# MasterBin-IIAU/Unicorn

Hardware: NVIDIA B200
Metric: frames/sec (higher is better)
Workload: dtype bf16

## Files before the change

### include/unicorn_b200.h

```cpp
#ifndef UNICORN_B200_H_
#define UNICORN_B200_H_
#include <stdint.h>

#ifdef __cplusplus
extern "C" {
#endif

#if defined(__GNUC__)
#define UC_API __attribute__((visibility("default")))
#else
#define UC_API
#endif

#define UC_OK 0
#define UC_EINVAL (-1)
#define UC_EDRIVER (-2)
#define UC_ENODEV (-3)

#define UC_BF16 0
#define UC_F32 1
#define UC_F16 2

#define UC_ACT_NONE 0
#define UC_ACT_RELU 1
// ... 19 lines not shown
  void* y;
  int ldy;
  int y_dtype;
  int block_n;
  void* gn_stats;
  int gn_groups;
  const void* row_stats;
  const float* col_s;
  float row_eps;
} UcConv2d;
UC_API int uc_conv2d(const UcConv2d* d, void* stream);

UC_API int uc_stem_ln(const void* img, int img_is_u8_hwc, const float* w48, const float* bias, const float* lnw, const float* lnb,
                      void* out_bf16, int B, int H, int W, int C0, float eps, void* stream);

UC_API int uc_dwconv7_ln(const void* x_bf16, const float* w49, const float* bias, const float* lnw, const float* lnb,
                         void* y_bf16, int B, int H, int W, int C, float eps, void* stream);

UC_API int uc_dwconv7(const void* x_bf16, const float* w49, const float* bias, void* y_bf16, int B, int H, int W, int C,
                      void* ln_stats, int* work_counter, void* stream);

UC_API int uc_dwconv7_mma(const void* x_bf16, const void* qtab, void* y_bf16, int B, int H, int W, int C, int* work_counter, void* stream);

UC_API int uc_convnext_mlp_supported(int C);
UC_API int uc_convnext_mlp(const void* t_bf16, const void* w1f_bf16, const float* c1, const void* w2_bf16, const float* b2, const float* gamma,
                           void* x_bf16, int M, int C, float ln_eps, void* stream);

UC_API int uc_layernorm(const void* x, int ldx, const void* res, int ldres, const float* w, const float* b, void* y,
                        int ldy, long M, int C, float eps, int dtype, void* stream);

UC_API int uc_groupnorm_apply(const void* x, int ldx, const void* stats, const float* w, const float* b, void* y,
                              int ldy, int B, long HW, int C, int G, float eps, int act, const float* prior,
                              const float* beta, const void* add2, int ldadd2, void* y2, int ldy2, void* stream);

UC_API int uc_copy_upsample(const void* src, int lds, void* dst, int ldd, int B, int Hs, int Ws, int C, int up, void* stream);
UC_API int uc_pixel_shuffle2(const void* in, int ldi, void* out, int ldo, int B, int H, int W, int Co, void* stream);
UC_API int uc_bilinear_f32(const float* src, float* dst, int P, int Hs, int Ws, int Hd, int Wd, float scale_h,
                           float scale_w, void* stream);
UC_API int uc_letterbox_u8(const uint8_t* src_hwc, int Hs, int Ws, uint8_t* dst_hwc, int Hd, int Wd, int rh, int rw,
                           int swap_rb, int pad, void* stream);
UC_API int uc_add(const void* a, int lda, const void* b, int ldb, void* y, int ldy, long M, int C, int dtype, void* stream);
UC_API int uc_copy_rows_if(const int* flag_dev, int invert, const void* src, long src_ld_bytes, void* dst, long dst_ld_bytes, long rows,
                           int row_bytes, void* stream);
UC_API int uc_nchw_f32_to_nhwc(const float* src, void* dst, int ldd, int B, int C, long HW, int dtype, void* stream);
UC_API int uc_nhwc_to_nchw_f32(const void* src, int lds, float* dst, int B, int C, long HW, int dtype, void* stream);

// ... 43 lines not shown
```

### unicorn_b200/csrc/conv_gemm.cu

```cuda
#include <algorithm>
#include <stdlib.h>
#include "uc_ptx.cuh"
#include "uc_common.h"
#include "../../include/unicorn_b200.h"
#include "uc_epilogue.cuh"

namespace uc {

constexpr int kBlockM = 128;
constexpr int kBlockK = 64;
constexpr int kMaxTaps = 9;
constexpr int kABytes = kBlockM * kBlockK * 2;
constexpr int kConvEpiWarps = 16;
constexpr int kConvThreads = (2 + kConvEpiWarps) * 32;
constexpr int kGnMaxLocal = 64;
constexpr int kGnSmemBytes = 2 * kGnMaxLocal * 2 * 8;

struct ConvTap {
  int16_t map, dw, dh, tap;
};

struct alignas(64) ConvKernelParams {
  CUtensorMap tmA[4];
  CUtensorMap tmB;
  CUtensorMap tmBh;
  ConvTap taps[kMaxTaps];
  int ntaps, kchunks;
  int n_tiles, m_tiles;
  int tile_w, tile_h, tiles_w, tiles_h;
  int Wo, Ho, B, Cout;
  uint32_t idesc;
  const float* bias;
  const float* gamma;
  const void* res;
  int ldres;
  void* y;
  int ldy, y_dtype, act;
  int wide_store, wide_res;
  int debug;
  const long long* row_stats;
  const float* col_s;
  float row_inv, row_eps;
  long long* gn_stats;
  int gn_groups, gn_gs;
};

__device__ __forceinline__ void gn_partial_sums(const float (&f)[16], const ConvKernelParams& p, int cbase, int ncols, bool valid,
                                             int lane, unsigned long long* acc_tile, int g0) {
  int c = 0;
#pragma unroll 1
  while (c < ncols) {
    const int g = (cbase + c) / p.gn_gs;
    const int end = min(ncols, (g + 1) * p.gn_gs - cbase);
    float s1 = 0.f, s2 = 0.f;
#pragma unroll
    for (int j = 0; j < 16; ++j) {
      const float x = (valid && j >= c && j < end) ? f[j] : 0.f;
      s1 += x;
      s2 = fmaf(x, x, s2);
    }
#pragma unroll
// ... 35 lines not shown
    prefetch_tmap(&p.tmA[0]);
    prefetch_tmap(&p.tmB);
    for (int i = 0; i < STAGES; ++i) {
      mbar_init(&full[i], 1);
      mbar_init(&empty[i], 1);
    }
    for (int i = 0; i < 2; ++i) {
      mbar_init(&tmem_full[i], 1);
      mbar_init(&tmem_empty[i], kConvEpiWarps * CLUSTER);
    }
    fence_barrier_init();
  }
  for (int i = threadIdx.x; i < 2 * kGnMaxLocal * 2; i += kConvThreads) gn_acc[i] = 0ull;
  if (warp == 1) {
    if (CLUSTER > 1) { tmem_alloc_2sm(tmem_slot, TMEM_COLS); tmem_relinquish_2sm(); }
    else { tmem_alloc(tmem_slot, TMEM_COLS); tmem_relinquish(); }
  }
  tc_fence_before();
  __syncthreads();
  if (CLUSTER > 1) cluster_sync_all();
  tc_fence_after();
  const uint32_t tmem_base = *tmem_slot;
  pdl_wait();
  pdl_launch_dependents();

  if (warp == 0) {
    int stage = 0, phase = 0;
    for (int item = item0; item < num_items; item += item_step) {
      const int n0 = (item % p.n_tiles) * BLOCK_N;
      const int mt = (item / p.n_tiles) * CLUSTER + crank;
      const int ow0 = (mt % p.tiles_w) * p.tile_w, oh0 = ((mt / p.tiles_w) % p.tiles_h) * p.tile_h;
      const int b = mt / (p.tiles_w * p.tiles_h);
      for (int t = 0; t < p.ntaps; ++t) {
        const ConvTap tp = p.taps[t];
        for (int kc = 0; kc < p.kchunks; ++kc) {
          mbar_wait(&empty[stage], phase ^ 1);
          if (elect_one()) {
            if (CLUSTER > 1 && p.debug == 2) {
              if (crank == 0) mbar_arrive(&full[stage]);
            } else if (CLUSTER > 1) {
              if (crank == 0) mbar_arrive_expect_tx(&full[stage], 2 * (kABytes + B_BYTES));
              tma_load_4d_2sm(sA + stage * kABytes, &p.tmA[tp.map], &full[stage], kc * kBlockK, ow0 + tp.dw, oh0 + tp.dh, b);
              tma_load_3d_2sm(sB + stage * B_BYTES, &p.tmBh, &full[stage], kc * kBlockK, tp.tap, n0 + crank * (BLOCK_N / 2));
            } else if (p.debug == 2) {
              mbar_arrive(&full[stage]);
            } else {
              mbar_arrive_expect_tx(&full[stage], kABytes + B_BYTES);
              tma_load_4d(sA + stage * kABytes, &p.tmA[tp.map], &full[stage], kc * kBlockK, ow0 + tp.dw, oh0 + tp.dh, b);
              tma_load_3d(sB + stage * B_BYTES, &p.tmB, &full[stage], kc * kBlockK, tp.tap, n0);
            }
          }
          __syncwarp();
          if (++stage == STAGES) { stage = 0; phase ^= 1; }
        }
      }
    }
  } else if (warp == 1) {
    if (crank == 0) {
      const uint32_t idesc = p.idesc;
      const uint64_t a_desc0 = umma_desc_sw128(smem_u32(sA)), b_desc0 = umma_desc_sw128(smem_u32(sB));
      int stage = 0, phase = 0, acc = 0, acc_phase = 0;
      for (int item = item0; item < num_items; item += item_step) {
        mbar_wait(&tmem_empty[acc], acc_phase ^ 1);
        tc_fence_after();
        const uint32_t d_tmem = tmem_base + acc * ACC_COLS;
        for (int it = 0; it < kiters; ++it) {
          mbar_wait(&full[stage], phase);
          tc_fence_after();
          if (CLUSTER == 1 && p.debug == 1) {
            if (elect_one()) {
              mbar_arrive(&empty[stage]);
              if (it == kiters - 1) mbar_arrive(&tmem_full[acc]);
            }
          } else if (elect_one()) {
            const uint64_t a_desc = a_desc0 + static_cast<uint64_t>((stage * kABytes) >> 4);
            const uint64_t b_desc = b_desc0 + static_cast<uint64_t>((stage * B_BYTES) >> 4);
#pragma unroll
            for (int k = 0; k < kBlockK / 16; ++k) {
              if (CLUSTER > 1) umma_f16_2sm(d_tmem, a_desc + 2 * k, b_desc + 2 * k, idesc, (it | k) != 0 ? 1u : 0u);
              else umma_f16(d_tmem, a_desc + 2 * k, b_desc + 2 * k, idesc, (it | k) != 0 ? 1u : 0u);
            }
            if (CLUSTER > 1) umma_commit_2sm_mc(&empty[stage], static_cast<uint16_t>(0x3));
            else umma_commit(&empty[stage]);
            if (it == kiters - 1) {
              if (CLUSTER > 1) umma_commit_2sm_mc(&tmem_full[acc], static_cast<uint16_t>(0x3));
              else umma_commit(&tmem_full[acc]);
            }
          }
          __syncwarp();
          if (++stage == STAGES) { stage = 0; phase ^= 1; }
        }
        acc ^= 1;
        if (acc == 0) acc_phase ^= 1;
      }
    }
  } else {
    const int q = warp & 3;
    const int cg = (warp - 2) >> 2;
    const int row = q * 32 + lane;
    const int wi = row % p.tile_w, hi = row / p.tile_w;
    const bool f16 = p.y_dtype == UC_F16;
    constexpr int ROUNDS = (BLOCK_N + 63) / 64;
    int acc = 0, acc_phase = 0, gpar = 0;
    for (int item = item0; item < num_items; item += item_step) {
      const int n0 = (item % p.n_tiles) * BLOCK_N;
      const int mt = (item / p.n_tiles) * CLUSTER + crank;
      const int ow0 = (mt % p.tiles_w) * p.tile_w, oh0 = ((mt / p.tiles_w) % p.tiles_h) * p.tile_h;
      const int b = mt / (p.tiles_w * p.tiles_h);
      const int ow = ow0 + wi, oh = oh0 + hi;
      const bool tile_ok = mt < p.m_tiles;
      const bool valid = (ow < p.Wo) && (oh < p.Ho) && tile_ok;
      const size_t pix = (static_cast<size_t>(b) * p.Ho + oh) * p.Wo + ow;
      const int limit = min(BLOCK_N, p.Cout - n0);
      float r_rstd = 1.f, r_murstd = 0.f;
      if (p.row_stats && valid) {
        const longlong2 st = __ldg(reinterpret_cast<const longlong2*>(p.row_stats) + pix);
        const float mu = static_cast<float>(st.x) * p.row_inv;
        const float var = fmaxf(fmaf(-mu, mu, static_cast<float>(st.y) * p.row_inv), 0.f);
        r_rstd = rsqrtf(var + p.row_eps);
        r_murstd = mu * r_rstd;
      }
      const int last_rd = (limit - 1 - cg * 16) >= 0 ? min(ROUNDS - 1, (limit - 1 - cg * 16) / 64) : -1;
      mbar_wait(&tmem_full[acc], acc_phase);
      tc_fence_after();
      const uint32_t t_acc = tmem_base + acc * ACC_COLS + (static_cast<uint32_t>(q * 32) << 16);
#pragma unroll 1
      for (int rd = 0; rd <= last_rd; ++rd) {
        const int c0 = rd * 64 + cg * 16;
        const int cbase = n0 + c0;
        const int ncols = min(16, limit - c0);
        uint32_t v[16];
        tmem_ld_32x16(t_acc + c0, v);
        float4 bb[4];
        if (p.bias) {
#pragma unroll
          for (int j = 0; j < 4; ++j) bb[j] = (4 * j < ncols) ? __ldg(reinterpret_cast<const float4*>(p.bias + cbase) + j) : make_float4(0.f, 0.f, 0.f, 0.f);
        } else {
#pragma unroll
          for (int j = 0; j < 4; ++j) bb[j] = make_float4(0.f, 0.f, 0.f, 0.f);
        }
        uint32_t rw[8];
        const bool has_res = p.res && valid;
        if (has_res) {
          const uint16_t* r = reinterpret_cast<const uint16_t*>(p.res) + pix * p.ldres + cbase;
          if (p.wide_res && ncols == 16) {
            ldg_v8(r, rw);
          } else {
// ... 283 lines not shown
  p.kchunks = (d->Cin + kBlockK - 1) / kBlockK;

  const int gn_gs = d->gn_stats ? d->Cout / d->gn_groups : 0;
  const bool cluster2 = d->block_n >= 1000;
  const int bn = cluster2 ? d->block_n - 1000 : d->block_n ? d->block_n : pick_block_n(d->Cout, m_tiles, gn_gs);
  if (bn == 0) return set_error(UC_EINVAL, "uc_conv2d: no N tile compatible with GroupNorm group size %d", gn_gs);
  {
    uint64_t dims[3] = {static_cast<uint64_t>(d->Cin), static_cast<uint64_t>(nt), static_cast<uint64_t>(d->Cout)};
    uint64_t strides[2] = {static_cast<uint64_t>(d->Cin) * es, static_cast<uint64_t>(nt) * d->Cin * es};
    uint32_t box[3] = {static_cast<uint32_t>(kBlockK), 1, static_cast<uint32_t>(bn)};
    rc = encode_tmap(&p.tmB, dt, 3, d->w, dims, strides, box);
    if (rc) return rc;
  }
  {
    const size_t yes = d->y_dtype == UC_F32 ? 4 : 2;
    p.wide_store = ((d->ldy * yes) % 32 == 0) && (reinterpret_cast<uintptr_t>(d->y) % 32 == 0);
    p.wide_res = d->res && ((d->ldres * es) % 32 == 0) && (reinterpret_cast<uintptr_t>(d->res) % 32 == 0);
  }
  p.Cout = d->Cout;
  {
    static int dbg = -1;
    if (dbg < 0) { const char* e = getenv("UC_CONV_DEBUG"); dbg = e ? atoi(e) : 0; }
    p.debug = dbg;
  }
  p.idesc = umma_idesc_f16(d->x_dtype == UC_BF16 ? 1u : 0u, kBlockM, static_cast<uint32_t>(bn));
  p.bias = d->bias; p.gamma = d->gamma; p.res = d->res; p.ldres = d->ldres;
  p.y = d->y; p.ldy = d->ldy; p.y_dtype = d->y_dtype; p.act = d->act;
  p.row_stats = static_cast<const long long*>(d->row_stats); p.col_s = d->col_s; p.row_inv = 1.f / (kGnFixedScale * static_cast<float>(d->Cin)); p.row_eps = d->row_eps;
  if (d->row_stats && (!d->col_s || d->KH != 1 || d->KW != 1 || d->stride != 1 || d->pad != 0))
    return set_error(UC_EINVAL, "uc_conv2d: row_stats (folded LayerNorm) needs a 1x1 stride-1 conv and col_s");
  p.gn_stats = static_cast<long long*>(d->gn_stats); p.gn_groups = d->gn_groups;
  p.gn_gs = d->gn_stats ? d->Cout / d->gn_groups : 1 << 30;
  if (d->gn_stats && (bn % p.gn_gs) != 0)
    return set_error(UC_EINVAL, "uc_conv2d: N tile %d incompatible with GroupNorm group size %d", bn, p.gn_gs);
  p.n_tiles = (d->Cout + bn - 1) / bn;
  p.m_tiles = m_tiles;
  if (cluster2) {
    uint64_t dims[3] = {static_cast<uint64_t>(d->Cin), static_cast<uint64_t>(nt), static_cast<uint64_t>(d->Cout)};
    uint64_t strides[2] = {static_cast<uint64_t>(d->Cin) * es, static_cast<uint64_t>(nt) * d->Cin * es};
    uint32_t box[3] = {static_cast<uint32_t>(kBlockK), 1, static_cast<uint32_t>(bn / 2)};
    rc = encode_tmap(&p.tmBh, dt, 3, d->w, dims, strides, box);
    if (rc) return rc;
    p.idesc = umma_idesc_f16(d->x_dtype == UC_BF16 ? 1u : 0u, 2 * kBlockM, static_cast<uint32_t>(bn));
    switch (bn) {
      case 256: return launch_conv<256, 6, 2>(p, stream);
      case 192: return launch_conv<192, 7, 2>(p, stream);
// ... 16 lines not shown
```

### unicorn_b200/csrc/dwconv_mma.cu

```cuda
#include "uc_ptx.cuh"
#include "uc_common.h"
#include "../../include/unicorn_b200.h"
#include <algorithm>
#include <stdlib.h>

namespace uc {

constexpr int kMmTW = 16, kMmTH = 16, kMmCH = 32;
constexpr int kMmHW = kMmTW + 8, kMmHH = kMmTH + 6;
constexpr int kMmPixBytes = kMmCH * 2;
constexpr int kMmStageBytes = kMmHH * kMmHW * kMmPixBytes;
constexpr int kMmPlaneBytes = kMmHH * kMmHW * 2;
constexpr int kMmPlanarBytes = kMmCH * kMmPlaneBytes;
constexpr int kMmPairBytes = kMmCH * 7 * 8 * 4;
constexpr int kMmQBytes = kMmPairBytes + kMmCH * 4;
constexpr int kMmSmem = kMmStageBytes + kMmPlanarBytes + kMmQBytes + 128 + 128;

struct alignas(64) DwMmaParams {
  CUtensorMap tmX;
  const uint8_t* qtab;
  uint16_t* y;
  int* work_counter;
  int H, W, C, B, tiles_w, tiles_h, n_items;
};

__device__ __forceinline__ int mm_plane(int c) { return (c & 7) * 4 + (c >> 3); }

__device__ __forceinline__ void bulk_load_1d(void* smem, const void* gmem, uint32_t bytes, uint64_t* bar) {
  asm volatile("cp.async.bulk.shared::cluster.global.mbarrier::complete_tx::bytes [%0], [%1], %2, [%3];" ::"r"(smem_u32(smem)), "l"(gmem),
               "r"(bytes), "r"(smem_u32(bar))
               : "memory");
}

struct DwFrag {
  uint32_t a[2][6];
  uint32_t q[2];
};

template <int NW>
__global__ void __launch_bounds__(NW * 32, NW == 4 ? 3 : 2) dwconv7_mma_kernel(const __grid_constant__ DwMmaParams p) {
  constexpr int CPW = kMmCH / NW;
  extern __shared__ uint8_t dsm_raw[];
  uint8_t* stage = dsm_raw + ((128u - (smem_u32(dsm_raw) & 127u)) & 127u);
  uint8_t* planar = stage + kMmStageBytes;
  uint8_t* qs = planar + kMmPlanarBytes;
  uint64_t* bar = reinterpret_cast<uint64_t*>(qs + kMmQBytes);
  volatile int* s_info = reinterpret_cast<volatile int*>(bar + 2);
  const int lane = threadIdx.x & 31, warp = threadIdx.x >> 5;
  const int g = lane >> 2, t = lane & 3;
  if (threadIdx.x == 0) {
    prefetch_tmap(&p.tmX);
    mbar_init(&bar[0], 1);
    mbar_init(&bar[1], 1);
    fence_barrier_init();
  }
  __syncthreads();
  pdl_wait();
  pdl_launch_dependents();
  const int tiles_img = p.tiles_w * p.tiles_h, tiles_chunk = tiles_img * p.B;
  int static_next = blockIdx.x;
// ... 3 lines not shown
    static_next += gridDim.x;
    return item;
  };
  auto issue = [&](int slot, int item) {
    volatile int* info = s_info + slot * 4;
    if (item >= p.n_items) {
      info[0] = -1;
      mbar_arrive(&bar[0]);
      return;
    }
    const int chunk = item / tiles_chunk, tt0 = item - chunk * tiles_chunk;
    const int b = tt0 / tiles_img, tt = tt0 - b * tiles_img;
    const int oh0 = (tt / p.tiles_w) * kMmTH, ow0 = (tt % p.tiles_w) * kMmTW;
    info[0] = chunk; info[1] = b; info[2] = oh0; info[3] = ow0;
    mbar_arrive_expect_tx(&bar[0], kMmStageBytes);
    tma_load_4d(stage, &p.tmX, &bar[0], chunk * kMmCH, ow0 - 4, oh0 - 3, b);
  };
  int pending = 0;
  if (threadIdx.x == 0) {
    issue(0, fetch());
    pending = fetch();
  }
  const int fc = warp * CPW;
  const uint32_t planar_w = smem_u32(planar) + mm_plane(fc) * kMmPlaneBytes;
  const uint32_t lm4 = planar_w + static_cast<uint32_t>((((lane & 7) + ((lane >> 3) & 1) * 8) * kMmHW + (lane >> 4) * 8) * 2);
  const uint32_t lm2 = planar_w + static_cast<uint32_t>(((lane & 15) * kMmHW + 16) * 2);
  const int d = 2 * t - g - 1;
  const bool first = d >= -1;
  const uint32_t q_lane = smem_u32(qs) + static_cast<uint32_t>((fc * 7 * 8 + (first ? d + 1 : d + 9)) * 4);
  const float* bias_s = reinterpret_cast<const float*>(qs + kMmPairBytes) + fc;
  const int tq = lane & 3, tsw = (lane >> 2) & 1;
  const uint32_t sel_lo = tsw ? 0x1054u : 0x5410u, sel_hi = tsw ? 0x3276u : 0x7632u;
  auto load_frag = [&](int s, DwFrag& f) {
    const int kh = s % 7;
#pragma unroll
    for (int j = 0; j < 2; ++j) {
      const int c = (s / 7) * 2 + j;
      const uint32_t off = static_cast<uint32_t>(c * 4 * kMmPlaneBytes + kh * (kMmHW * 2));
      asm volatile("ldmatrix.sync.aligned.m8n8.x4.shared.b16 {%0,%1,%2,%3}, [%4];"
                   : "=r"(f.a[j][0]), "=r"(f.a[j][1]), "=r"(f.a[j][2]), "=r"(f.a[j][3]) : "r"(lm4 + off));
      asm volatile("ldmatrix.sync.aligned.m8n8.x2.shared.b16 {%0,%1}, [%2];" : "=r"(f.a[j][4]), "=r"(f.a[j][5]) : "r"(lm2 + off));
      asm volatile("ld.shared.b32 %0, [%1];" : "=r"(f.q[j]) : "r"(q_lane + static_cast<uint32_t>((c * 7 + kh) * 32)));
    }
  };
  int prev_chunk = -1;
  uint32_t q_phase = 0;
  for (int it = 0;; ++it) {
    mbar_wait(&bar[0], it & 1);
    const int chunk = s_info[(it & 1) * 4 + 0];
    if (chunk < 0) break;
    const int b = s_info[(it & 1) * 4 + 1], oh0 = s_info[(it & 1) * 4 + 2], ow0 = s_info[(it & 1) * 4 + 3];
    const int c0 = chunk * kMmCH + fc;
    const bool new_chunk = chunk != prev_chunk;
    prev_chunk = chunk;
    if (new_chunk && threadIdx.x == 0) {
      mbar_arrive_expect_tx(&bar[1], kMmQBytes);
      bulk_load_1d(qs, p.qtab + static_cast<size_t>(chunk) * kMmQBytes, kMmQBytes, &bar[1]);
    }
    {
      const uint4* st = reinterpret_cast<const uint4*>(stage);
#pragma unroll 3
      for (int pp = warp * 8 + (lane >> 2); pp < kMmHH * kMmHW / 2; pp += NW * 8) {
        const uint4 va = st[(2 * pp + tsw) * 4 + tq];
        const uint4 vb = st[(2 * pp + (tsw ^ 1)) * 4 + tq];
        const uint32_t wa[4] = {va.x, va.y, va.z, va.w}, wb[4] = {vb.x, vb.y, vb.z, vb.w};
        uint8_t* dst = planar + pp * 4;
#pragma unroll
        for (int j = 0; j < 8; ++j)
          *reinterpret_cast<uint32_t*>(dst + mm_plane(tq * 8 + j) * kMmPlaneBytes) = __byte_perm(wa[j >> 1], wb[j >> 1], j & 1 ? sel_hi : sel_lo);
      }
    }
    __syncthreads();
    if (threadIdx.x == 0) {
      issue((it + 1) & 1, pending);
      pending = fetch();
    }
    if (new_chunk) {
      mbar_wait(&bar[1], q_phase);
      q_phase ^= 1;
    }
    if (c0 < p.C) {
      float acc[CPW][2][4];
#pragma unroll
      for (int c = 0; c < CPW; ++c) {
        const float bv = bias_s[c];
#pragma unroll
        for (int e = 0; e < 4; ++e) acc[c][0][e] = acc[c][1][e] = bv;
      }
      DwFrag fr[2];
      load_frag(0, fr[0]);
#pragma unroll
      for (int s = 0; s < CPW / 2 * 7; ++s) {
        if (s + 1 < CPW / 2 * 7) load_frag(s + 1, fr[(s + 1) & 1]);
        const DwFrag& f = fr[s & 1];
#pragma unroll
        for (int j = 0; j < 2; ++j) {
          const int c = (s / 7) * 2 + j;
          const uint32_t b0 = first ? f.q[j] : 0u, b1 = first ? 0u : f.q[j];
#pragma unroll
          for (int nb = 0; nb < 2; ++nb)
            asm volatile("mma.sync.aligned.m16n8k16.row.col.f32.bf16.bf16.f32 {%0,%1,%2,%3}, {%4,%5,%6,%7}, {%8,%9}, {%0,%1,%2,%3};"
                         : "+f"(acc[c][nb][0]), "+f"(acc[c][nb][1]), "+f"(acc[c][nb][2]), "+f"(acc[c][nb][3])
                         : "r"(f.a[j][2 * nb]), "r"(f.a[j][2 * nb + 1]), "r"(f.a[j][2 * nb + 2]), "r"(f.a[j][2 * nb + 3]), "r"(b0), "r"(b1));
        }
      }
      uint16_t* yb = p.y + ((static_cast<size_t>(b) * p.H + oh0) * p.W + ow0) * p.C + c0;
#pragma unroll
      for (int nb = 0; nb < 2; ++nb)
#pragma unroll
        for (int e = 0; e < 4; ++e) {
          const int r = g + (e >> 1) * 8, cl = nb * 8 + 2 * t + (e & 1);
          if (oh0 + r < p.H && ow0 + cl < p.W) {
            uint16_t* dst = yb + (static_cast<size_t>(r) * p.W + cl) * p.C;
            if constexpr (CPW == 8) {
              uint4 o;
              o.x = pack_bf16(acc[0][nb][e], acc[1][nb][e]); o.y = pack_bf16(acc[2][nb][e], acc[3][nb][e]);
              o.z = pack_bf16(acc[4][nb][e], acc[5][nb][e]); o.w = pack_bf16(acc[6][nb][e], acc[7][nb][e]);
              *reinterpret_cast<uint4*>(dst) = o;
            } else {
              *reinterpret_cast<uint2*>(dst) = make_uint2(pack_bf16(acc[0][nb][e], acc[1][nb][e]), pack_bf16(acc[2][nb][e], acc[3][nb][e]));
            }
          }
        }
    }
    __syncthreads();
  }
}

}

using namespace uc;

extern "C" int uc_dwconv7_mma(const void* x_bf16, const void* qtab, void* y_bf16, int B, int H, int W, int C,
                              int* work_counter, void* stream_v) {
  cudaStream_t stream = static_cast<cudaStream_t>(stream_v);
  if (!x_bf16 || !qtab || !y_bf16) return set_error(UC_EINVAL, "uc_dwconv7_mma: null pointer");
  if (x_bf16 == y_bf16) return set_error(UC_EINVAL, "uc_dwconv7_mma: not an in-place operation");
  if (B < 1 || H < 1 || W < 1 || C < 8 || C % 8) return set_error(UC_EINVAL, "uc_dwconv7_mma: C must be a multiple of 8");
  if ((reinterpret_cast<uintptr_t>(x_bf16) | reinterpret_cast<uintptr_t>(y_bf16) | reinterpret_cast<uintptr_t>(qtab)) & 15) return set_error(UC_EINVAL, "uc_dwconv7_mma: 16-byte aligned maps");
  int rc = ensure_driver();
  if (rc) return rc;
  DwMmaParams p;
  memset(&p, 0, sizeof(p));
  {
    uint64_t dims[4] = {static_cast<uint64_t>(C), static_cast<uint64_t>(W), static_cast<uint64_t>(H), static_cast<uint64_t>(B)};
    uint64_t strides[3] = {static_cast<uint64_t>(C) * 2, static_cast<uint64_t>(W) * C * 2, static_cast<uint64_t>(H) * W * C * 2};
    uint32_t box[4] = {kMmCH, kMmHW, kMmHH, 1};
    rc = encode_tmap(&p.tmX, CU_TENSOR_MAP_DATA_TYPE_BFLOAT16, 4, x_bf16, dims, strides, box, CU_TENSOR_MAP_SWIZZLE_NONE);
// ... 5 lines not shown
  p.H = H; p.W = W; p.C = C; p.B = B;
  p.tiles_w = (W + kMmTW - 1) / kMmTW;
  p.tiles_h = (H + kMmTH - 1) / kMmTH;
  const long items = static_cast<long>(p.tiles_w) * p.tiles_h * B * ((C + kMmCH - 1) / kMmCH);
  if (items > 0x7fffffffL) return set_error(UC_EINVAL, "uc_dwconv7_mma: too many tiles");
  p.n_items = static_cast<int>(items);
  static int forced = -1;
  if (forced < 0) { const char* e = getenv("UC_DW_MMA_WARPS"); forced = e ? atoi(e) : 0; }
  const bool wide = forced == 8;
  static PerDeviceFlag attr_dev;
  bool& attr = attr_dev.get();
  if (!attr) {
    cudaError_t e = cudaFuncSetAttribute(dwconv7_mma_kernel<4>, cudaFuncAttributeMaxDynamicSharedMemorySize, kMmSmem);
    if (e == cudaSuccess) e = cudaFuncSetAttribute(dwconv7_mma_kernel<8>, cudaFuncAttributeMaxDynamicSharedMemorySize, kMmSmem);
    if (e != cudaSuccess) return set_error(static_cast<int>(e), "uc_dwconv7_mma: cudaFuncSetAttribute: %s", cudaGetErrorString(e));
    attr = true;
  }
  const int grid = static_cast<int>(std::min<long>(items, static_cast<long>(num_sms()) * (wide ? 2 : 3)));
  cudaError_t e = wide ? launch_pdl(dwconv7_mma_kernel<8>, dim3(grid), dim3(256), kMmSmem, stream, p)
                       : launch_pdl(dwconv7_mma_kernel<4>, dim3(grid), dim3(128), kMmSmem, stream, p);
  if (e != cudaSuccess) return set_error(static_cast<int>(e), "uc_dwconv7_mma launch: %s", cudaGetErrorString(e));
  return check_launch("uc_dwconv7_mma");
}
```

### unicorn_b200/engine.py

```python
import os

import torch

from . import ops
from .weights import CONFIGS

ACT_NONE, ACT_RELU, ACT_GELU, ACT_SILU = ops.ACT_NONE, ops.ACT_RELU, ops.ACT_GELU, ops.ACT_SILU
BF16, F16, F32 = torch.bfloat16, torch.float16, torch.float32
STRIDES = (8, 16, 32)


class _ConvGN:

    def __init__(self, w, gw, gb, k, stride, groups=16, eps=1e-3, bias=None):
        self.w, self.gw, self.gb, self.k, self.stride, self.groups, self.eps, self.bias = w, gw, gb, k, stride, groups, eps, bias
        self.cout = w.shape[0]


class UnicornEngine:
    def __init__(self, state_dict, cfg_name, device="cuda", autotune=True, ln_fold=None):
        ops._lib.check(ops._lib.lib().uc_check_device(), "uc_check_device")
        self.cfg_name = cfg_name
        self.cfg = CONFIGS[cfg_name]
        self.dev = torch.device(device)
        self.dims = self.cfg["dims"]
        self.depths = self.cfg["depths"]
        self.ncls = self.cfg["num_classes"]
        self._bufs = {}
        self._stats_arena = None
        self._stats_used = 0
        self._pos_cache = {}
        self._side_streams = None
        self._fork_stream = None
        self._with_masks = False
        self._bn_cache = {}
        self._bn_dirty = False
        self.ln_fold = bool(int(os.environ.get("UC_LN_FOLD", "0"))) if ln_fold is None else bool(ln_fold)
        self.dw_mma = bool(int(os.environ.get("UC_DW_MMA", "1")))
        self.mlp_fused = bool(int(os.environ.get("UC_MLP_FUSED", "1")))
        self.mlp_min_rows = int(os.environ.get("UC_MLP_MIN_ROWS", "0"))
        self._row_arena, self._row_used = None, 0
        self._ctr_arena, self._ctr_used = None, 0
        self.autotune = autotune
        self.load_tuning()
        self._load(state_dict)

    def fork(self):
        import copy
        ctx = copy.copy(self)
        ctx._bufs = {}
        ctx._stats_arena, ctx._stats_used = None, 0
        ctx._row_arena, ctx._row_used = None, 0
        ctx._ctr_arena, ctx._ctr_used = None, 0
        ctx._side_streams, ctx._fork_stream = None, None
        return ctx

    def _load(self, sd):
        dev = self.dev
        f = lambda k: sd[k].to(dev, F32).contiguous()
        pw = lambda k: ops.pack_conv_weight(sd[k].to(dev, F32))
        P = {}
# ... 213 lines not shown
        band_mb = float(os.environ.get("UC_MLP_BAND_MB", "0"))
        nb = 1
        if band_mb > 0 and B == 1:
            nb = max(1, -(-(H * W * 4 * C * 2) // int(band_mb * 2 ** 20)))
            while H % nb:
                nb += 1
        hb = H // nb
        if bp.get("fused") and (C != 256 or B * H * W >= self.mlp_min_rows):
            if self.dw_mma:
                t = ops.dwconv7_mma(x, bp["dwm"], out=self.buf(tag + ".t", x.shape), work_counter=self._ctr())
            else:
                t = ops.dwconv7(x, bp["dw"], bp["dwb"], out=self.buf(tag + ".t", x.shape), work_counter=self._ctr())
            ops.convnext_mlp(t.view(-1, C), bp["w1f"], bp["c1"], bp["w2"], bp["b2"], bp["gamma"], x.view(-1, C), 1e-6)
            return x
        hid = self.buf(tag + ".h", (B, hb, W, 4 * C))
        if self.ln_fold and C % 32 == 0:
            rs = self._row_stats(B * H * W)
            t = ops.dwconv7(x, bp["dw"], bp["dwb"], out=self.buf(tag + ".t", x.shape), ln_stats=rs, work_counter=self._ctr())
            for i in range(nb):
                xs, ts = x[:, i * hb:(i + 1) * hb], t[:, i * hb:(i + 1) * hb]
                self.conv(ts, bp["w1f"], 1, bias=bp["c1"], act=ACT_GELU, out=hid, row_stats=rs[i * hb * W:(i + 1) * hb * W], col_s=bp["s1"], row_eps=1e-6)
                self.conv(hid, bp["w2"], 1, bias=bp["b2"], gamma=bp["gamma"], res=xs, out=xs)
            return x
        if self.dw_mma and C % 8 == 0:
            t = ops.dwconv7_mma(x, bp["dwm"], out=self.buf(tag + ".t", x.shape), work_counter=self._ctr())
        else:
            t = ops.dwconv7(x, bp["dw"], bp["dwb"], out=self.buf(tag + ".t", x.shape), work_counter=self._ctr())
        ops.layernorm(t.view(-1, C), bp["lnw"], bp["lnb"], 1e-6, out=t.view(-1, C))
        for i in range(nb):
            xs, ts = x[:, i * hb:(i + 1) * hb], t[:, i * hb:(i + 1) * hb]
            self.conv(ts, bp["w1"], 1, bias=bp["b1"], act=ACT_GELU, out=hid)
            self.conv(hid, bp["w2"], 1, bias=bp["b2"], gamma=bp["gamma"], res=xs, out=xs)
        return x

    def csp(self, x, cp, out, tag):
        B, H, W, _ = x.shape
        hdim = cp["c12"].cout // 2
        cat = self.buf(tag + ".cat", (B, H, W, 2 * hdim))
        self.conv_gn(x, cp["c12"], cat)
        cur = cat[..., :hdim]
        for i, (c1, c2) in enumerate(cp["m"]):
            t = self.conv_gn(cur, c1, self.buf(tag + ".m1", (B, H, W, hdim)))
            dst = cat[..., :hdim] if i == len(cp["m"]) - 1 else self.buf(tag + f".m2_{i % 2}", (B, H, W, hdim))
            cur = self.conv_gn(t, c2, dst)
        return self.conv_gn(cat, cp["c3"], out)

    def backbone(self, img, tag="cur", side=None):
        feats, seq = self.features(img, tag)
        if side is None:
            return self.neck(feats, tag), seq
        main = torch.cuda.current_stream()
# ... 191 lines not shown
```

### unicorn_b200/ops.py

```python
import ctypes

import torch

from . import _lib
from ._lib import BF16, F32, F16, ACT_NONE, ACT_RELU, ACT_GELU, ACT_SILU, ACT_SIGMOID

_DT = {torch.bfloat16: BF16, torch.float32: F32, torch.float16: F16}


def _p(t):
    return ctypes.c_void_p(t.data_ptr()) if t is not None else None


def _nhwc_ld(t):
    assert t.dim() == 4 and t.is_cuda, "expected a CUDA NHWC tensor"
    B, H, W, C = t.shape
    ld = t.stride(2) if W > 1 else (t.stride(1) // W if H > 1 else max(C, t.stride(2)))
    assert t.stride(3) == 1 or C == 1
    if W > 1:
        assert t.stride(2) == ld
    if H > 1:
        assert t.stride(1) == W * ld, (t.shape, t.stride())
    if B > 1:
        assert t.stride(0) == H * W * ld
# ... 86 lines not shown


def pack_dw_weight_mma(w, bias):
    C = w.shape[0]
    Cp = -(-C // 32) * 32
    e = torch.zeros(Cp, 7, 9, dtype=torch.bfloat16, device=w.device)
    e[:C, :, 1:8] = w.reshape(C, 7, 7).to(torch.bfloat16)
    bits = e.view(torch.int16).to(torch.int32) & 0xffff
    pairs = (bits[:, :, 0:8] | (bits[:, :, 1:9] << 16)).to(torch.int32).reshape(Cp // 32, 32 * 7 * 8)
    bp = torch.zeros(Cp, dtype=torch.float32, device=w.device)
    bp[:C] = bias.float()
    return torch.cat([pairs, bp.view(torch.int32).reshape(Cp // 32, 32)], dim=1).contiguous()


def dwconv7_mma(x, qtab, out=None, work_counter=None):
    B, H, W, C = x.shape
    assert x.is_contiguous() and x.dtype == torch.bfloat16 and qtab.dtype == torch.int32 and qtab.shape == (-(-C // 32), 1824)
    if out is None:
        out = torch.empty_like(x)
    _lib.check(_L().uc_dwconv7_mma(_p(x), _p(qtab), _p(out), B, H, W, C, _p(work_counter), _S()), "uc_dwconv7_mma")
    return out


def convnext_mlp_supported(C):
    return bool(_L().uc_convnext_mlp_supported(int(C)))


def convnext_mlp(t, w1f, c1, w2, b2, gamma, x, eps=1e-6):
    M, C = t.shape
    assert t.is_contiguous() and x.is_contiguous() and x.shape == t.shape and t.dtype == x.dtype == torch.bfloat16
    assert w1f.dtype == torch.bfloat16 and w1f.numel() == 4 * C * C and w2.dtype == torch.bfloat16 and w2.numel() == 4 * C * C
    _lib.check(_L().uc_convnext_mlp(_p(t), _p(w1f), _p(c1), _p(w2), _p(b2), _p(gamma), _p(x), M, C, ctypes.c_float(eps), _S()), "uc_convnext_mlp")
    return x


def stem_ln(img, w48, bias, lnw, lnb, eps=1e-6):
    u8 = img.dtype == torch.uint8
    if u8:
        B, H, W, _ = img.shape
    else:
        B, _, H, W = img.shape
        assert img.dtype == torch.float32
    assert img.is_contiguous()
    C0 = w48.shape[1]
    out = torch.empty(B, H // 4, W // 4, C0, dtype=torch.bfloat16, device=img.device)
    _lib.check(_L().uc_stem_ln(_p(img), int(u8), _p(w48), _p(bias), _p(lnw), _p(lnb), _p(out), B, H, W, C0, _f(eps), _S()), "uc_stem_ln")
# ... 243 lines not shown
```

Baseline: 297.3.

## Add cluster-fused dwconv7+LayerNorm kernel and late PDL trigger in conv GEMM

Result: no change. 298.2 (median of 6 runs) (+0.3%).

```diff
diff --git a/include/unicorn_b200.h b/include/unicorn_b200.h
--- a/include/unicorn_b200.h
+++ b/include/unicorn_b200.h
@@ -65,6 +65,10 @@
 
 UC_API int uc_dwconv7_mma(const void* x_bf16, const void* qtab, void* y_bf16, int B, int H, int W, int C, int* work_counter, void* stream);
 
+UC_API int uc_dwconv7_mma_ln_supported(int C);
+UC_API int uc_dwconv7_mma_ln(const void* x_bf16, const void* qtab, const float* lnw, const float* lnb, void* y_bf16, int B, int H, int W,
+                             int C, float eps, void* stream);
+
 UC_API int uc_convnext_mlp_supported(int C);
 UC_API int uc_convnext_mlp(const void* t_bf16, const void* w1f_bf16, const float* c1, const void* w2_bf16, const float* b2, const float* gamma,
                            void* x_bf16, int M, int C, float ln_eps, void* stream);
diff --git a/unicorn_b200/csrc/conv_gemm.cu b/unicorn_b200/csrc/conv_gemm.cu
--- a/unicorn_b200/csrc/conv_gemm.cu
+++ b/unicorn_b200/csrc/conv_gemm.cu
@@ -37,6 +37,7 @@
   void* y;
   int ldy, y_dtype, act;
   int wide_store, wide_res;
+  int pdl_late;
   int debug;
   const long long* row_stats;
   const float* col_s;
@@ -118,7 +119,7 @@
   tc_fence_after();
   const uint32_t tmem_base = *tmem_slot;
   pdl_wait();
-  pdl_launch_dependents();
+  if (!p.pdl_late) pdl_launch_dependents();
 
   if (warp == 0) {
     int stage = 0, phase = 0;
@@ -151,6 +152,7 @@
         }
       }
     }
+    if (p.pdl_late) pdl_launch_dependents();
   } else if (warp == 1) {
     if (crank == 0) {
       const uint32_t idesc = p.idesc;
@@ -190,6 +192,7 @@
         if (acc == 0) acc_phase ^= 1;
       }
     }
+    if (p.pdl_late) pdl_launch_dependents();
   } else {
     const int q = warp & 3;
     const int cg = (warp - 2) >> 2;
@@ -219,6 +222,7 @@
       const int last_rd = (limit - 1 - cg * 16) >= 0 ? min(ROUNDS - 1, (limit - 1 - cg * 16) / 64) : -1;
       mbar_wait(&tmem_full[acc], acc_phase);
       tc_fence_after();
+      if (p.pdl_late && item + item_step >= num_items) pdl_launch_dependents();
       const uint32_t t_acc = tmem_base + acc * ACC_COLS + (static_cast<uint32_t>(q * 32) << 16);
 #pragma unroll 1
       for (int rd = 0; rd <= last_rd; ++rd) {
@@ -548,6 +552,9 @@
     static int dbg = -1;
     if (dbg < 0) { const char* e = getenv("UC_CONV_DEBUG"); dbg = e ? atoi(e) : 0; }
     p.debug = dbg;
+    static int late = -1;
+    if (late < 0) { const char* e = getenv("UC_CONV_PDL_LATE"); late = e ? atoi(e) : 1; }
+    p.pdl_late = late;
   }
   p.idesc = umma_idesc_f16(d->x_dtype == UC_BF16 ? 1u : 0u, kBlockM, static_cast<uint32_t>(bn));
   p.bias = d->bias; p.gamma = d->gamma; p.res = d->res; p.ldres = d->ldres;
diff --git a/unicorn_b200/csrc/dwconv_mma.cu b/unicorn_b200/csrc/dwconv_mma.cu
--- a/unicorn_b200/csrc/dwconv_mma.cu
+++ b/unicorn_b200/csrc/dwconv_mma.cu
@@ -36,6 +36,81 @@
   uint32_t a[2][6];
   uint32_t q[2];
 };
+
+template <int NW>
+__device__ __forceinline__ void mm_transpose(const uint8_t* stage, uint8_t* planar, int warp, int lane) {
+  const int tq = lane & 3, tsw = (lane >> 2) & 1;
+  const uint32_t sel_lo = tsw ? 0x1054u : 0x5410u, sel_hi = tsw ? 0x3276u : 0x7632u;
+  const uint4* st = reinterpret_cast<const uint4*>(stage);
+#pragma unroll 3
+  for (int pp = warp * 8 + (lane >> 2); pp < kMmHH * kMmHW / 2; pp += NW * 8) {
+    const uint4 va = st[(2 * pp + tsw) * 4 + tq];
+    const uint4 vb = st[(2 * pp + (tsw ^ 1)) * 4 + tq];
+    const uint32_t wa[4] = {va.x, va.y, va.z, va.w}, wb[4] = {vb.x, vb.y, vb.z, vb.w};
+    uint8_t* dst = planar + pp * 4;
+#pragma unroll
+    for (int j = 0; j < 8; ++j)
+      *reinterpret_cast<uint32_t*>(dst + mm_plane(tq * 8 + j) * kMmPlaneBytes) = __byte_perm(wa[j >> 1], wb[j >> 1], j & 1 ? sel_hi : sel_lo);
+  }
+}
+
+struct DwLane {
+  uint32_t lm4, lm2;
+  uint32_t q_off;
+  bool first;
+};
+
+__device__ __forceinline__ DwLane mm_lane(const uint8_t* planar, int fc, int lane) {
+  const int g = lane >> 2, t = lane & 3;
+  DwLane L;
+  const uint32_t planar_w = smem_u32(planar) + mm_plane(fc) * kMmPlaneBytes;
+  L.lm4 = planar_w + static_cast<uint32_t>((((lane & 7) + ((lane >> 3) & 1) * 8) * kMmHW + (lane >> 4) * 8) * 2);
+  L.lm2 = planar_w + static_cast<uint32_t>(((lane & 15) * kMmHW + 16) * 2);
+  const int d = 2 * t - g - 1;
+  L.first = d >= -1;
+  L.q_off = static_cast<uint32_t>((fc * 7 * 8 + (L.first ? d + 1 : d + 9)) * 4);
+  return L;
+}
+
+template <int CPW>
+__device__ __forceinline__ void mm_dw_tile(const DwLane& L, uint32_t q_base, const float* bias_s, float (&acc)[CPW][2][4]) {
+  const uint32_t q_lane = q_base + L.q_off;
+  auto load_frag = [&](int s, DwFrag& f) {
+    const int kh = s % 7;
+#pragma unroll
+    for (int j = 0; j < 2; ++j) {
+      const int c = (s / 7) * 2 + j;
+      const uint32_t off = static_cast<uint32_t>(c * 4 * kMmPlaneBytes + kh * (kMmHW * 2));
+      asm volatile("ldmatrix.sync.aligned.m8n8.x4.shared.b16 {%0,%1,%2,%3}, [%4];"
+                   : "=r"(f.a[j][0]), "=r"(f.a[j][1]), "=r"(f.a[j][2]), "=r"(f.a[j][3]) : "r"(L.lm4 + off));
+      asm volatile("ldmatrix.sync.aligned.m8n8.x2.shared.b16 {%0,%1}, [%2];" : "=r"(f.a[j][4]), "=r"(f.a[j][5]) : "r"(L.lm2 + off));
+      asm volatile("ld.shared.b32 %0, [%1];" : "=r"(f.q[j]) : "r"(q_lane + static_cast<uint32_t>((c * 7 + kh) * 32)));
+    }
+  };
+#pragma unroll
+  for (int c = 0; c < CPW; ++c) {
+    const float bv = bias_s[c];
+#pragma unroll
+    for (int e = 0; e < 4; ++e) acc[c][0][e] = acc[c][1][e] = bv;
+  }
+  DwFrag fr[2];
+  load_frag(0, fr[0]);
+#pragma unroll
+  for (int s = 0; s < CPW / 2 * 7; ++s) {
+    if (s + 1 < CPW / 2 * 7) load_frag(s + 1, fr[(s + 1) & 1]);
+    const DwFrag& f = fr[s & 1];
+#pragma unroll
+    for (int j = 0; j < 2; ++j) {
+      const int c = (s / 7) * 2 + j;
+      const uint32_t b0 = L.first ? f.q[j] : 0u, b1 = L.first ? 0u : f.q[j];
+#pragma unroll
+      for (int nb = 0; nb < 2; ++nb)
+        asm volatile("mma.sync.aligned.m16n8k16.row.col.f32.bf16.bf16.f32 {%0,%1,%2,%3}, {%4,%5,%6,%7}, {%8,%9}, {%0,%1,%2,%3};"
+                     : "+f"(acc[c][nb][0]), "+f"(acc[c][nb][1]), "+f"(acc[c][nb][2]), "+f"(acc[c][nb][3])
+                     : "r"(f.a[j][2 * nb]), "r"(f.a[j][2 * nb + 1]), "r"(f.a[j][2 * nb + 2]), "r"(f.a[j][2 * nb + 3]), "r"(b0), "r"(b1));
+    }
+  }
+}
 
 template <int NW>
 __global__ void __launch_bounds__(NW * 32, NW == 4 ? 3 : 2) dwconv7_mma_kernel(const __grid_constant__ DwMmaParams p) {
@@ -85,27 +160,8 @@
     pending = fetch();
   }
   const int fc = warp * CPW;
-  const uint32_t planar_w = smem_u32(planar) + mm_plane(fc) * kMmPlaneBytes;
-  const uint32_t lm4 = planar_w + static_cast<uint32_t>((((lane & 7) + ((lane >> 3) & 1) * 8) * kMmHW + (lane >> 4) * 8) * 2);
-  const uint32_t lm2 = planar_w + static_cast<uint32_t>(((lane & 15) * kMmHW + 16) * 2);
-  const int d = 2 * t - g - 1;
-  const bool first = d >= -1;
-  const uint32_t q_lane = smem_u32(qs) + static_cast<uint32_t>((fc * 7 * 8 + (first ? d + 1 : d + 9)) * 4);
+  const DwLane L = mm_lane(planar, fc, lane);
   const float* bias_s = reinterpret_cast<const float*>(qs + kMmPairBytes) + fc;
-  const int tq = lane & 3, tsw = (lane >> 2) & 1;
-  const uint32_t sel_lo = tsw ? 0x1054u : 0x5410u, sel_hi = tsw ? 0x3276u : 0x7632u;
-  auto load_frag = [&](int s, DwFrag& f) {
-    const int kh = s % 7;
-#pragma unroll
-    for (int j = 0; j < 2; ++j) {
-      const int c = (s / 7) * 2 + j;
-      const uint32_t off = static_cast<uint32_t>(c * 4 * kMmPlaneBytes + kh * (kMmHW * 2));
-      asm volatile("ldmatrix.sync.aligned.m8n8.x4.shared.b16 {%0,%1,%2,%3}, [%4];"
-                   : "=r"(f.a[j][0]), "=r"(f.a[j][1]), "=r"(f.a[j][2]), "=r"(f.a[j][3]) : "r"(lm4 + off));
-      asm volatile("ldmatrix.sync.aligned.m8n8.x2.shared.b16 {%0,%1}, [%2];" : "=r"(f.a[j][4]), "=r"(f.a[j][5]) : "r"(lm2 + off));
-      asm volatile("ld.shared.b32 %0, [%1];" : "=r"(f.q[j]) : "r"(q_lane + static_cast<uint32_t>((c * 7 + kh) * 32)));
-    }
-  };
   int prev_chunk = -1;
   uint32_t q_phase = 0;
   for (int it = 0;; ++it) {
@@ -120,19 +176,7 @@
       mbar_arrive_expect_tx(&bar[1], kMmQBytes);
       bulk_load_1d(qs, p.qtab + static_cast<size_t>(chunk) * kMmQBytes, kMmQBytes, &bar[1]);
     }
-    {
-      const uint4* st = reinterpret_cast<const uint4*>(stage);
-#pragma unroll 3
-      for (int pp = warp * 8 + (lane >> 2); pp < kMmHH * kMmHW / 2; pp += NW * 8) {
-        const uint4 va = st[(2 * pp + tsw) * 4 + tq];
-        const uint4 vb = st[(2 * pp + (tsw ^ 1)) * 4 + tq];
-        const uint32_t wa[4] = {va.x, va.y, va.z, va.w}, wb[4] = {vb.x, vb.y, vb.z, vb.w};
-        uint8_t* dst = planar + pp * 4;
-#pragma unroll
-        for (int j = 0; j < 8; ++j)
-          *reinterpret_cast<uint32_t*>(dst + mm_plane(tq * 8 + j) * kMmPlaneBytes) = __byte_perm(wa[j >> 1], wb[j >> 1], j & 1 ? sel_hi : sel_lo);
-      }
-    }
+    mm_transpose<NW>(stage, planar, warp, lane);
     __syncthreads();
     if (threadIdx.x == 0) {
       issue((it + 1) & 1, pending);
@@ -144,29 +188,7 @@
     }
     if (c0 < p.C) {
       float acc[CPW][2][4];
-#pragma unroll
-      for (int c = 0; c < CPW; ++c) {
-        const float bv = bias_s[c];
-#pragma unroll
-        for (int e = 0; e < 4; ++e) acc[c][0][e] = acc[c][1][e] = bv;
-      }
-      DwFrag fr[2];
-      load_frag(0, fr[0]);
-#pragma unroll
-      for (int s = 0; s < CPW / 2 * 7; ++s) {
-        if (s + 1 < CPW / 2 * 7) load_frag(s + 1, fr[(s + 1) & 1]);
-        const DwFrag& f = fr[s & 1];
-#pragma unroll
-        for (int j = 0; j < 2; ++j) {
-          const int c = (s / 7) * 2 + j;
-          const uint32_t b0 = first ? f.q[j] : 0u, b1 = first ? 0u : f.q[j];
-#pragma unroll
-          for (int nb = 0; nb < 2; ++nb)
-            asm volatile("mma.sync.aligned.m16n8k16.row.col.f32.bf16.bf16.f32 {%0,%1,%2,%3}, {%4,%5,%6,%7}, {%8,%9}, {%0,%1,%2,%3};"
-                         : "+f"(acc[c][nb][0]), "+f"(acc[c][nb][1]), "+f"(acc[c][nb][2]), "+f"(acc[c][nb][3])
-                         : "r"(f.a[j][2 * nb]), "r"(f.a[j][2 * nb + 1]), "r"(f.a[j][2 * nb + 2]), "r"(f.a[j][2 * nb + 3]), "r"(b0), "r"(b1));
-        }
-      }
+      mm_dw_tile<CPW>(L, smem_u32(qs), bias_s, acc);
       uint16_t* yb = p.y + ((static_cast<size_t>(b) * p.H + oh0) * p.W + ow0) * p.C + c0;
 #pragma unroll
       for (int nb = 0; nb < 2; ++nb)
@@ -187,6 +209,182 @@
         }
     }
     __syncthreads();
+  }
+}
+
+constexpr int kLnNch = 3;
+constexpr int kLnPix = kMmTH * kMmTW;
+constexpr int kLnQBytes = kLnNch * kMmQBytes;
+__host__ __device__ constexpr int dwln_smem(int CL) {
+  return kMmStageBytes + kMmPlanarBytes + kLnQBytes + 2 * CL * kLnPix * 4 + 128 + 128;
+}
+
+struct alignas(64) DwLnParams {
+  CUtensorMap tmX;
+  const uint8_t* qtab;
+  const float* lnw;
+  const float* lnb;
+  uint16_t* y;
+  int H, W, C, tiles_w, tiles_h;
+  float eps;
+};
+
+__device__ __forceinline__ void cluster_arrive_relaxed() { asm volatile("barrier.cluster.arrive.relaxed.aligned;" ::: "memory"); }
+__device__ __forceinline__ void cluster_arrive_release() { asm volatile("barrier.cluster.arrive.release.aligned;" ::: "memory"); }
+__device__ __forceinline__ void cluster_wait_acquire() { asm volatile("barrier.cluster.wait.acquire.aligned;" ::: "memory"); }
+__device__ __forceinline__ void st_cluster_f32x2(uint32_t local_addr, uint32_t rank, float a, float b) {
+  asm volatile(
+      "{\n\t.reg .b32 ra;\n\t"
+      "mapa.shared::cluster.u32 ra, %0, %1;\n\t"
+      "st.shared::cluster.v2.f32 [ra], {%2, %3};\n\t}" ::"r"(local_addr), "r"(rank), "f"(a), "f"(b)
+      : "memory");
+}
+
+template <int CL, bool RSTD>
+__device__ __forceinline__ void dwln_round(const float (&lp)[2][4], float* wpart, float* part, float* out, uint32_t rank, float c_count,
+                                           float eps, int warp, int lane) {
+  const int g = lane >> 2, t = lane & 3;
+#pragma unroll
+  for (int nb = 0; nb < 2; ++nb)
+#pragma unroll
+    for (int e = 0; e < 4; ++e) wpart[warp * kLnPix + (g + (e >> 1) * 8) * kMmTW + nb * 8 + 2 * t + (e & 1)] = lp[nb][e];
+  __syncthreads();
+  const int p0 = 2 * threadIdx.x;
+  const float2 w0 = *reinterpret_cast<const float2*>(wpart + p0), w1 = *reinterpret_cast<const float2*>(wpart + kLnPix + p0);
+  const float2 w2 = *reinterpret_cast<const float2*>(wpart + 2 * kLnPix + p0), w3 = *reinterpret_cast<const float2*>(wpart + 3 * kLnPix + p0);
+  const float a = ((w0.x + w1.x) + w2.x) + w3.x, b = ((w0.y + w1.y) + w2.y) + w3.y;
+  const uint32_t slot = smem_u32(part + rank * kLnPix + p0);
+#pragma unroll
+  for (int q = 0; q < CL; ++q) st_cluster_f32x2(slot, static_cast<uint32_t>(q), a, b);
+  cluster_arrive_release();
+  cluster_wait_acquire();
+  float sa = 0.f, sb = 0.f;
+#pragma unroll
+  for (int q = 0; q < CL; ++q) {
+    const float2 v = *reinterpret_cast<const float2*>(part + q * kLnPix + p0);
+    sa += v.x;
+    sb += v.y;
+  }
+  sa /= c_count;
+  sb /= c_count;
+  if (RSTD) {
+    sa = rsqrtf(sa + eps);
+    sb = rsqrtf(sb + eps);
+  }
+  *reinterpret_cast<float2*>(out + p0) = make_float2(sa, sb);
+  __syncthreads();
+}
+
+template <int CL>
+__global__ void __launch_bounds__(128, 2) dwconv7_mma_ln_kernel(const __grid_constant__ DwLnParams p) {
+  extern __shared__ uint8_t dsm_raw[];
+  uint8_t* stage = dsm_raw + ((128u - (smem_u32(dsm_raw) & 127u)) & 127u);
+  uint8_t* planar = stage + kMmStageBytes;
+  uint8_t* qs = planar + kMmPlanarBytes;
+  float* part1 = reinterpret_cast<float*>(qs + kLnQBytes);
+  float* part2 = part1 + CL * kLnPix;
+  uint64_t* bar = reinterpret_cast<uint64_t*>(part2 + CL * kLnPix);
+  float* wpart = reinterpret_cast<float*>(stage);
+  float* s_mean = wpart + 4 * kLnPix;
+  float* s_rstd = s_mean + kLnPix;
+  const int lane = threadIdx.x & 31, warp = threadIdx.x >> 5;
+  const int g = lane >> 2, t = lane & 3;
+  const uint32_t rank = cluster_ctarank();
+  const int tile = blockIdx.x / CL;
+  const int tiles_img = p.tiles_w * p.tiles_h;
+  const int b = tile / tiles_img, tt = tile - b * tiles_img;
+  const int oh0 = (tt / p.tiles_w) * kMmTH, ow0 = (tt % p.tiles_w) * kMmTW;
+  const int chunk0 = static_cast<int>(rank) * kLnNch;
+  if (threadIdx.x == 0) {
+    prefetch_tmap(&p.tmX);
+    mbar_init(&bar[0], 1);
+    mbar_init(&bar[1], 1);
+    fence_barrier_init();
+  }
+  cluster_arrive_relaxed();
+  __syncthreads();
+  pdl_wait();
+  if (threadIdx.x == 0) {
+    mbar_arrive_expect_tx(&bar[1], kLnQBytes);
+    bulk_load_1d(qs, p.qtab + static_cast<size_t>(chunk0) * kMmQBytes, kLnQBytes, &bar[1]);
+    mbar_arrive_expect_tx(&bar[0], kMmStageBytes);
+    tma_load_4d(stage, &p.tmX, &bar[0], chunk0 * kMmCH, ow0 - 4, oh0 - 3, b);
+  }
+  const int fc = warp * 8;
+  const DwLane L = mm_lane(planar, fc, lane);
+  uint32_t v[kLnNch][2][4][4];
+  float lp[2][4];
+#pragma unroll
+  for (int nb = 0; nb < 2; ++nb)
+#pragma unroll
+    for (int e = 0; e < 4; ++e) lp[nb][e] = 0.f;
+#pragma unroll
+  for (int k = 0; k < kLnNch; ++k) {
+    mbar_wait(&bar[0], k & 1);
+    mm_transpose<4>(stage, planar, warp, lane);
+    __syncthreads();
+    if (k + 1 < kLnNch && threadIdx.x == 0) {
+      mbar_arrive_expect_tx(&bar[0], kMmStageBytes);
+      tma_load_4d(stage, &p.tmX, &bar[0], (chunk0 + k + 1) * kMmCH, ow0 - 4, oh0 - 3, b);
+    }
+    if (k == 0) mbar_wait(&bar[1], 0);
+    float acc[8][2][4];
+    mm_dw_tile<8>(L, smem_u32(qs + k * kMmQBytes), reinterpret_cast<const float*>(qs + k * kMmQBytes + kMmPairBytes) + fc, acc);
+#pragma unroll
+    for (int nb = 0; nb < 2; ++nb)
+#pragma unroll
+      for (int e = 0; e < 4; ++e)
+#pragma unroll
+        for (int c = 0; c < 4; ++c) {
+          const uint32_t w = pack_bf16(acc[2 * c][nb][e], acc[2 * c + 1][nb][e]);
+          v[k][nb][e][c] = w;
+          lp[nb][e] += bf16lo(w) + bf16hi(w);
+        }
+    if (k + 1 < kLnNch) __syncthreads();
+  }
+  cluster_wait_acquire();
+  pdl_launch_dependents();
+  const float fC = static_cast<float>(p.C);
+  dwln_round<CL, false>(lp, wpart, part1, s_mean, rank, fC, p.eps, warp, lane);
+#pragma unroll
+  for (int nb = 0; nb < 2; ++nb)
+#pragma unroll
+    for (int e = 0; e < 4; ++e) {
+      const float mu = s_mean[(g + (e >> 1) * 8) * kMmTW + nb * 8 + 2 * t + (e & 1)];
+      float q = 0.f;
+#pragma unroll
+      for (int k = 0; k < kLnNch; ++k)
+#pragma unroll
+        for (int c = 0; c < 4; ++c) {
+          const float d0 = bf16lo(v[k][nb][e][c]) - mu, d1 = bf16hi(v[k][nb][e][c]) - mu;
+          q = fmaf(d0, d0, q);
+          q = fmaf(d1, d1, q);
+        }
+      lp[nb][e] = q;
+    }
+  dwln_round<CL, true>(lp, wpart, part2, s_rstd, rank, fC, p.eps, warp, lane);
+#pragma unroll
+  for (int k = 0; k < kLnNch; ++k) {
+    const int c0 = (chunk0 + k) * kMmCH + fc;
+    const float4 w0 = __ldg(reinterpret_cast<const float4*>(p.lnw + c0)), w1 = __ldg(reinterpret_cast<const float4*>(p.lnw + c0 + 4));
+    const float4 b0 = __ldg(reinterpret_cast<const float4*>(p.lnb + c0)), b1 = __ldg(reinterpret_cast<const float4*>(p.lnb + c0 + 4));
+    const float ww[8] = {w0.x, w0.y, w0.z, w0.w, w1.x, w1.y, w1.z, w1.w}, bb[8] = {b0.x, b0.y, b0.z, b0.w, b1.x, b1.y, b1.z, b1.w};
+    uint16_t* yb = p.y + ((static_cast<size_t>(b) * p.H + oh0) * p.W + ow0) * p.C + c0;
+#pragma unroll
+    for (int nb = 0; nb < 2; ++nb)
+#pragma unroll
+      for (int e = 0; e < 4; ++e) {
+        const int r = g + (e >> 1) * 8, cl = nb * 8 + 2 * t + (e & 1);
+        if (oh0 + r < p.H && ow0 + cl < p.W) {
+          const float mu = s_mean[r * kMmTW + cl], rs = s_rstd[r * kMmTW + cl];
+          uint32_t o[4];
+#pragma unroll
+          for (int c = 0; c < 4; ++c)
+            o[c] = pack_bf16((bf16lo(v[k][nb][e][c]) - mu) * rs * ww[2 * c] + bb[2 * c],
+                             (bf16hi(v[k][nb][e][c]) - mu) * rs * ww[2 * c + 1] + bb[2 * c + 1]);
+          *reinterpret_cast<uint4*>(yb + (static_cast<size_t>(r) * p.W + cl) * p.C) = make_uint4(o[0], o[1], o[2], o[3]);
+        }
+      }
   }
 }
 
@@ -238,3 +436,71 @@
   if (e != cudaSuccess) return set_error(static_cast<int>(e), "uc_dwconv7_mma launch: %s", cudaGetErrorString(e));
   return check_launch("uc_dwconv7_mma");
 }
+
+static int dwln_cluster(int C) { return C == 768 ? 8 : 0; }
+
+extern "C" int uc_dwconv7_mma_ln_supported(int C) { return dwln_cluster(C) != 0; }
+
+template <int CL>
+static int launch_dwln_cluster(const DwLnParams& p, int tiles, cudaStream_t stream) {
+  constexpr int smem = dwln_smem(CL);
+  static PerDeviceFlag attr_dev;
+  bool& attr = attr_dev.get();
+  if (!attr) {
+    cudaError_t e = cudaFuncSetAttribute(dwconv7_mma_ln_kernel<CL>, cudaFuncAttributeMaxDynamicSharedMemorySize, smem);
+    if (e != cudaSuccess) return set_error(static_cast<int>(e), "uc_dwconv7_mma_ln: cudaFuncSetAttribute: %s", cudaGetErrorString(e));
+    attr = true;
+  }
+  cudaLaunchConfig_t cfg = {};
+  cfg.gridDim = dim3(static_cast<unsigned>(tiles) * CL);
+  cfg.blockDim = dim3(128);
+  cfg.dynamicSmemBytes = smem;
+  cfg.stream = stream;
+  cudaLaunchAttribute attrs[2];
+  attrs[0].id = cudaLaunchAttributeClusterDimension;
+  attrs[0].val.clusterDim.x = CL;
+  attrs[0].val.clusterDim.y = 1;
+  attrs[0].val.clusterDim.z = 1;
+  attrs[1].id = cudaLaunchAttributeProgrammaticStreamSerialization;
+  attrs[1].val.programmaticStreamSerializationAllowed = 1;
+  cfg.attrs = attrs;
+  cfg.numAttrs = pdl_enabled() ? 2 : 1;
+  const cudaError_t e = cudaLaunchKernelEx(&cfg, dwconv7_mma_ln_kernel<CL>, p);
+  if (e != cudaSuccess) return set_error(static_cast<int>(e), "uc_dwconv7_mma_ln launch: %s", cudaGetErrorString(e));
+  return check_launch("uc_dwconv7_mma_ln");
+}
+
+extern "C" int uc_dwconv7_mma_ln(const void* x_bf16, const void* qtab, const float* lnw, const float* lnb, void* y_bf16, int B, int H,
+                                 int W, int C, float eps, void* stream_v) {
+  cudaStream_t stream = static_cast<cudaStream_t>(stream_v);
+  if (!x_bf16 || !qtab || !lnw || !lnb || !y_bf16) return set_error(UC_EINVAL, "uc_dwconv7_mma_ln: null pointer");
+  if (x_bf16 == y_bf16) return set_error(UC_EINVAL, "uc_dwconv7_mma_ln: not an in-place operation");
+  if (B < 1 || H < 1 || W < 1 || C < 8 || C % 8) return set_error(UC_EINVAL, "uc_dwconv7_mma_ln: C must be a multiple of 8");
+  if ((reinterpret_cast<uintptr_t>(x_bf16) | reinterpret_cast<uintptr_t>(y_bf16) | reinterpret_cast<uintptr_t>(qtab) |
+       reinterpret_cast<uintptr_t>(lnw) | reinterpret_cast<uintptr_t>(lnb)) & 15)
+    return set_error(UC_EINVAL, "uc_dwconv7_mma_ln: 16-byte aligned maps and vectors");
+  const int CL = dwln_cluster(C);
+  if (!CL) return set_error(UC_EINVAL, "uc_dwconv7_mma_ln: C not supported (768)");
+  int rc = ensure_driver();
+  if (rc) return rc;
+  DwLnParams p;
+  memset(&p, 0, sizeof(p));
+  {
+    uint64_t dims[4] = {static_cast<uint64_t>(C), static_cast<uint64_t>(W), static_cast<uint64_t>(H), static_cast<uint64_t>(B)};
+    uint64_t strides[3] = {static_cast<uint64_t>(C) * 2, static_cast<uint64_t>(W) * C * 2, static_cast<uint64_t>(H) * W * C * 2};
+    uint32_t box[4] = {kMmCH, kMmHW, kMmHH, 1};
+    rc = encode_tmap(&p.tmX, CU_TENSOR_MAP_DATA_TYPE_BFLOAT16, 4, x_bf16, dims, strides, box, CU_TENSOR_MAP_SWIZZLE_NONE);
+    if (rc) return rc;
+  }
+  p.qtab = static_cast<const uint8_t*>(qtab);
+  p.lnw = lnw;
+  p.lnb = lnb;
+  p.y = static_cast<uint16_t*>(y_bf16);
+  p.H = H; p.W = W; p.C = C;
+  p.tiles_w = (W + kMmTW - 1) / kMmTW;
+  p.tiles_h = (H + kMmTH - 1) / kMmTH;
+  p.eps = eps;
+  const long tiles = static_cast<long>(p.tiles_w) * p.tiles_h * B;
+  if (tiles * CL > 0x7fffffffL) return set_error(UC_EINVAL, "uc_dwconv7_mma_ln: too many tiles");
+  return launch_dwln_cluster<8>(p, static_cast<int>(tiles), stream);
+}
diff --git a/unicorn_b200/engine.py b/unicorn_b200/engine.py
--- a/unicorn_b200/engine.py
+++ b/unicorn_b200/engine.py
@@ -37,6 +37,7 @@
         self._bn_dirty = False
         self.ln_fold = bool(int(os.environ.get("UC_LN_FOLD", "0"))) if ln_fold is None else bool(ln_fold)
         self.dw_mma = bool(int(os.environ.get("UC_DW_MMA", "1")))
+        self.dw_ln_cluster = bool(int(os.environ.get("UC_DW_LN_CLUSTER", "0")))
         self.mlp_fused = bool(int(os.environ.get("UC_MLP_FUSED", "1")))
         self.mlp_min_rows = int(os.environ.get("UC_MLP_MIN_ROWS", "0"))
         self._row_arena, self._row_used = None, 0
@@ -296,11 +297,14 @@
                 self.conv(ts, bp["w1f"], 1, bias=bp["c1"], act=ACT_GELU, out=hid, row_stats=rs[i * hb * W:(i + 1) * hb * W], col_s=bp["s1"], row_eps=1e-6)
                 self.conv(hid, bp["w2"], 1, bias=bp["b2"], gamma=bp["gamma"], res=xs, out=xs)
             return x
-        if self.dw_mma and C % 8 == 0:
-            t = ops.dwconv7_mma(x, bp["dwm"], out=self.buf(tag + ".t", x.shape), work_counter=self._ctr())
+        if self.dw_mma and self.dw_ln_cluster and ops.dwconv7_mma_ln_supported(C):
+            t = ops.dwconv7_mma_ln(x, bp["dwm"], bp["lnw"], bp["lnb"], 1e-6, out=self.buf(tag + ".t", x.shape))
         else:
-            t = ops.dwconv7(x, bp["dw"], bp["dwb"], out=self.buf(tag + ".t", x.shape), work_counter=self._ctr())
-        ops.layernorm(t.view(-1, C), bp["lnw"], bp["lnb"], 1e-6, out=t.view(-1, C))
+            if self.dw_mma and C % 8 == 0:
+                t = ops.dwconv7_mma(x, bp["dwm"], out=self.buf(tag + ".t", x.shape), work_counter=self._ctr())
+            else:
+                t = ops.dwconv7(x, bp["dw"], bp["dwb"], out=self.buf(tag + ".t", x.shape), work_counter=self._ctr())
+            ops.layernorm(t.view(-1, C), bp["lnw"], bp["lnb"], 1e-6, out=t.view(-1, C))
         for i in range(nb):
             xs, ts = x[:, i * hb:(i + 1) * hb], t[:, i * hb:(i + 1) * hb]
             self.conv(ts, bp["w1"], 1, bias=bp["b1"], act=ACT_GELU, out=hid)
diff --git a/unicorn_b200/ops.py b/unicorn_b200/ops.py
--- a/unicorn_b200/ops.py
+++ b/unicorn_b200/ops.py
@@ -132,6 +132,20 @@
     return out
 
 
+def dwconv7_mma_ln_supported(C):
+    return bool(_L().uc_dwconv7_mma_ln_supported(int(C)))
+
+
+def dwconv7_mma_ln(x, qtab, lnw, lnb, eps=1e-6, out=None):
+    B, H, W, C = x.shape
+    assert x.is_contiguous() and x.dtype == torch.bfloat16 and qtab.dtype == torch.int32 and qtab.shape == (-(-C // 32), 1824)
+    assert lnw.dtype == lnb.dtype == torch.float32 and lnw.numel() == lnb.numel() == C and lnw.is_contiguous() and lnb.is_contiguous()
+    if out is None:
+        out = torch.empty_like(x)
+    _lib.check(_L().uc_dwconv7_mma_ln(_p(x), _p(qtab), _p(lnw), _p(lnb), _p(out), B, H, W, C, _f(eps), _S()), "uc_dwconv7_mma_ln")
+    return out
+
+
 def convnext_mlp_supported(C):
     return bool(_L().uc_convnext_mlp_supported(int(C)))
 
```
